# jianzhnie/ScaleRL

Measured on NVIDIA H100. Metric: learner_frames_per_sec, higher is better.
Workload: dtype bf16

## Files before the change

scalerl_b200/csrc/igemm_tma.cuh:

```cuda
#pragma once
#include <cuda.h>
#include "common.cuh"
#include "kernels.h"

namespace srl {

SRL_DEVINL void tma_prefetch_desc(const CUtensorMap* m) {
  asm volatile("prefetch.tensormap [%0];" ::"l"(reinterpret_cast<uint64_t>(m)) : "memory");
}
SRL_DEVINL void tma_load_2d(void* dst, const CUtensorMap* m, uint64_t* bar, int c0, int c1) {
  asm volatile("cp.async.bulk.tensor.2d.shared::cluster.global.mbarrier::complete_tx::bytes [%0], [%1, {%3, %4}], [%2];"
               ::"r"(smem_u32(dst)), "l"(reinterpret_cast<uint64_t>(m)), "r"(smem_u32(bar)), "r"(c0), "r"(c1) : "memory");
}
SRL_DEVINL void tma_load_3d(void* dst, const CUtensorMap* m, uint64_t* bar, int c0, int c1, int c2) {
  asm volatile("cp.async.bulk.tensor.3d.shared::cluster.global.mbarrier::complete_tx::bytes [%0], [%1, {%3, %4, %5}], [%2];"
               ::"r"(smem_u32(dst)), "l"(reinterpret_cast<uint64_t>(m)), "r"(smem_u32(bar)), "r"(c0), "r"(c1), "r"(c2) : "memory");
}
SRL_DEVINL void tma_load_4d(void* dst, const CUtensorMap* m, uint64_t* bar, int c0, int c1, int c2, int c3) {
  asm volatile("cp.async.bulk.tensor.4d.shared::cluster.global.mbarrier::complete_tx::bytes [%0], [%1, {%3, %4, %5, %6}], [%2];"
               ::"r"(smem_u32(dst)), "l"(reinterpret_cast<uint64_t>(m)), "r"(smem_u32(bar)), "r"(c0), "r"(c1), "r"(c2), "r"(c3)
               : "memory");
}
SRL_DEVINL void tma_load_5d(void* dst, const CUtensorMap* m, uint64_t* bar, int c0, int c1, int c2, int c3, int c4) {
  asm volatile("cp.async.bulk.tensor.5d.shared::cluster.global.mbarrier::complete_tx::bytes [%0], [%1, {%3, %4, %5, %6, %7}], [%2];"
               ::"r"(smem_u32(dst)), "l"(reinterpret_cast<uint64_t>(m)), "r"(smem_u32(bar)), "r"(c0), "r"(c1), "r"(c2), "r"(c3), "r"(c4)
               : "memory");
}

constexpr int IGT_THREADS = 288;

template <class P, int SPLIT = 0>
struct TmaCfg {
  static constexpr int KROWS = P::A_MN ? P::KROWS : 64;
  static constexpr int A_BYTES = P::A_MN ? 2 * KROWS * 128 : 128 * 128;
  static constexpr int B_BLOCKS = (P::BN + 63) / 64;
  static constexpr int B_BYTES = P::B_MN ? B_BLOCKS * KROWS * 128 : P::BN * 128;
  static constexpr int HALF_BYTES = A_BYTES + B_BYTES;
  static constexpr int STAGE_BYTES = HALF_BYTES * (1 + SPLIT);
  static constexpr int NB = P::BN / 2;
  static constexpr int STAGES = fit_stages(P::STAGES, 2 * WG_IMG_BYTES + 1024 + 256, STAGE_BYTES);
  static constexpr int SMEM_BYTES = STAGES * STAGE_BYTES + 2 * WG_IMG_BYTES + 1024 + 256;
  static_assert(SMEM_BYTES <= 232448, "shared memory budget (227 KB)");
  static_assert(NB == 32 || NB == 64 || NB == 128, "MMA N per warpgroup");
  static constexpr int MMAS = P::A_MN ? KROWS / 16 : 4;
  static_assert(A_BYTES % 1024 == 0 && B_BYTES % 1024 == 0, "operand tiles must keep 1024 B alignment (SWIZZLE_128B atoms)");
  static_assert(P::A_MN == P::B_MN, "mixed majors are not used");
  static_assert(KROWS % 16 == 0, "contraction rows per stage must be a multiple of MMA K = 16");
};

template <class P, int SPLIT>
SRL_DEVINL void igt_epilogue(const typename P::Params& p, int tm, int ty, int row, int c0, float (&v)[16]) {
  if constexpr (SPLIT) P::template epilogue16<1>(p, tm, ty, row, c0, v); else P::epilogue16(p, tm, ty, row, c0, v);
}
template <class P, int SPLIT>
SRL_DEVINL void igt_epilogue(const typename P::Params& p, int tm, int ty, int row, int c0, float (&v)[16], const uint4 (&pre)[2]) {
  if constexpr (SPLIT) P::template epilogue16<1>(p, tm, ty, row, c0, v, pre); else P::epilogue16(p, tm, ty, row, c0, v, pre);
}

template <class P, int SPLIT = 0>
__global__ void __launch_bounds__(IGT_THREADS) igemm_tma_kernel(const __grid_constant__ typename P::Params p) {
  using C = TmaCfg<P, SPLIT>;
  extern __shared__ uint8_t smem_raw[];
  uint8_t* smem = reinterpret_cast<uint8_t*>((reinterpret_cast<uintptr_t>(smem_raw) + 1023) & ~uintptr_t(1023));
  float* img = reinterpret_cast<float*>(smem + C::STAGES * C::STAGE_BYTES);
  uint64_t* bars = reinterpret_cast<uint64_t*>(smem + C::STAGES * C::STAGE_BYTES + 2 * WG_IMG_BYTES);
  uint64_t* full = bars;
  uint64_t* empty = bars + C::STAGES;

  const int tid = threadIdx.x;
  const int warp = tid >> 5;
  const int tm = blockIdx.x, ty = blockIdx.y;
  const int nkb = P::num_kblocks(p, tm, ty);

  if constexpr (P::ZERO_INIT) {
    if (P::zero_cta(ty)) {
      uint4* z = reinterpret_cast<uint4*>(smem);
      for (int i = tid; i < C::STAGES * C::STAGE_BYTES / 16; i += IGT_THREADS) z[i] = make_uint4(0, 0, 0, 0);
    }
    __syncthreads();
    for (int s = 0; s < C::STAGES; ++s) P::init_smem(p, tm, ty, smem + s * C::STAGE_BYTES, tid);
    fence_proxy_async_smem();
  }
  if (warp == 8 && (tid & 31) == 0) {
    for (int s = 0; s < C::STAGES; ++s) { mbar_init(&full[s], 1); mbar_init(&empty[s], 8); }
    mbar_fence_init();
    P::prefetch(p);
  }
  __syncthreads();
  pdl_wait(P::KID);
  if (tid == 256) pdl_launch();

  if (warp == 8) {
    const uint32_t leader = elect_one_sync();
    for (int kb = 0; kb < nkb; ++kb) {
      const int s = kb % C::STAGES;
      mbar_wait(&empty[s], ((kb / C::STAGES) & 1) ^ 1);
      if (leader) {
        uint8_t* sA = smem + s * C::STAGE_BYTES;
        if constexpr (SPLIT) P::issue_split(p, tm, ty, kb, sA, C::A_BYTES, C::HALF_BYTES, &full[s]);
        else P::issue(p, tm, ty, kb, sA, sA + C::A_BYTES, &full[s]);
      }
      __syncwarp();
    }
  } else {
    const int g = warp >> 2, wt = tid & 127;
    constexpr int NB = C::NB;
    uint4 pre[P::PREFETCH ? NB / 16 : 1][2];
    if constexpr (P::PREFETCH) {
#pragma unroll
      for (int c = 0; c < NB / 16; ++c) P::prefetch16(p, tm, ty, wt, g * NB + c * 16, pre[c]);
    }
    float acc[2][NB / 2];
#pragma unroll
    for (int h = 0; h < 2; ++h)
#pragma unroll
      for (int i = 0; i < NB / 2; ++i) acc[h][i] = 0.f;
    constexpr uint32_t ASTEP = P::A_MN ? 2048 / 16 : 32 / 16, BSTEP = P::B_MN ? 2048 / 16 : 32 / 16;
    constexpr uint32_t A_HI = (P::A_MN ? C::KROWS * 128 : 64 * 128) / 16;
    const uint32_t b_off = P::B_MN ? (g * NB / 64) * C::KROWS * 128 + (g * NB % 64) * 2 : g * NB * 128;
    for (int kb = 0; kb < nkb; ++kb) {
      const int s = kb % C::STAGES;
      mbar_wait(&full[s], (kb / C::STAGES) & 1);
      const uint32_t a0 = smem_u32(smem + s * C::STAGE_BYTES);
      const uint64_t ad0 = P::A_MN ? make_smem_desc(a0, C::KROWS * 128, 1024) : make_smem_desc(a0, 16, 1024);
      const uint64_t bd0 = P::B_MN ? make_smem_desc(a0 + C::A_BYTES + b_off, C::KROWS * 128, 1024) : make_smem_desc(a0 + C::A_BYTES + b_off, 16, 1024);
      wg_fence();
#pragma unroll
      for (int k = 0; k < C::MMAS; ++k) {
        const uint64_t ad = ad0 + (uint64_t)(k * ASTEP), bd = bd0 + (uint64_t)(k * BSTEP);
        wg_mma128<NB, P::A_MN ? 1 : 0, P::B_MN ? 1 : 0>(acc, ad, A_HI, bd, (kb | k) != 0);
        if constexpr (SPLIT) {
          wg_mma128<NB, P::A_MN ? 1 : 0, P::B_MN ? 1 : 0>(acc, ad, A_HI, bd + (uint64_t)(C::HALF_BYTES / 16), 1);
          wg_mma128<NB, P::A_MN ? 1 : 0, P::B_MN ? 1 : 0>(acc, ad + (uint64_t)(C::HALF_BYTES / 16), A_HI, bd, 1);
        }
      }
      wg_commit();
      if constexpr (C::STAGES > 1) {
        wg_wait_prev();
        __syncwarp();
        if (kb > 0 && (tid & 31) == 0) mbar_arrive(&empty[(kb - 1) % C::STAGES]);
      } else {
        wg_wait_all();
        __syncwarp();
        if ((tid & 31) == 0) mbar_arrive(&empty[s]);
      }
    }
    wg_wait_all();
    wg_fence_regs(acc[0]); wg_fence_regs(acc[1]);
    float* my_img = img + g * (WG_IMG_BYTES / 4);
#pragma unroll
    for (int c = 0; c < NB / 16; ++c) {
      float v[16];
      wg_acc_row16<NB>(acc, c, my_img, wt, 2 + g, v);
      if constexpr (P::PREFETCH) igt_epilogue<P, SPLIT>(p, tm, ty, wt, g * NB + c * 16, v, pre[c]);
      else igt_epilogue<P, SPLIT>(p, tm, ty, wt, g * NB + c * 16, v);
    }
  }
}

template <class P, int SPLIT = 0>
cudaError_t igemm_tma_launch(const typename P::Params& p, dim3 grid, cudaStream_t stream) {
  using C = TmaCfg<P, SPLIT>;
  if (grid.x == 0 || grid.y == 0) return cudaSuccess;
  static PerDeviceOnce once;
  { cudaError_t e = ensure_max_dynamic_smem(once, igemm_tma_kernel<P, SPLIT>, C::SMEM_BYTES); if (e != cudaSuccess) return e; }
  return launch_chain(igemm_tma_kernel<P, SPLIT>, grid, dim3(IGT_THREADS), C::SMEM_BYTES, stream, p);
}

}
```

scalerl_b200/csrc/tma_problems.cuh:

```cuda
#pragma once
#include "igemm_tma.cuh"
#include "encoder_problems.cuh"

namespace srl {

#define SRL_TMAP alignas(64) CUtensorMap

struct TFcFwd {
  static constexpr int KID = 31;
  static constexpr bool PREFETCH = false;
  static constexpr int BN = 64, STAGES = 4, SPLITS = 4;
  static constexpr bool A_MN = false, B_MN = false, ZERO_INIT = false;
  static constexpr int KROWS = 64;
  struct Params { SRL_TMAP a3m; SRL_TMAP w; SRL_TMAP a3m_lo; SRL_TMAP w_lo; float* out; int M; };
  SRL_DEVINL static void prefetch(const Params& p) { tma_prefetch_desc(&p.a3m); tma_prefetch_desc(&p.w); }
  SRL_DEVINL static int kb_begin(int split) { return (49 * split) / SPLITS; }
  SRL_DEVINL static void issue_split(const Params& p, int tm, int ty, int kb, uint8_t* st, int a_bytes, int half, uint64_t* bar) {
    const int k = (kb_begin(ty % SPLITS) + kb) * 64;
    mbar_arrive_expect_tx(bar, 2 * (128 * 128 + 64 * 128));
    tma_load_2d(st, &p.a3m, bar, k, tm * 128);
    tma_load_2d(st + a_bytes, &p.w, bar, k, (ty / SPLITS) * 64);
    tma_load_2d(st + half, &p.a3m_lo, bar, k, tm * 128);
    tma_load_2d(st + half + a_bytes, &p.w_lo, bar, k, (ty / SPLITS) * 64);
  }
  template <int SPLIT>
  SRL_DEVINL static void epilogue16(const Params& p, int tm, int ty, int row, int c0, float (&v)[16]) { epilogue16(p, tm, ty, row, c0, v); }
  SRL_DEVINL static int num_kblocks(const Params&, int, int ty) { const int sp = ty % SPLITS; return kb_begin(sp + 1) - kb_begin(sp); }
  SRL_DEVINL static void issue(const Params& p, int tm, int ty, int kb, uint8_t* sA, uint8_t* sB, uint64_t* bar) {
    const int k = (kb_begin(ty % SPLITS) + kb) * 64;
    mbar_arrive_expect_tx(bar, 128 * 128 + 64 * 128);
    tma_load_2d(sA, &p.a3m, bar, k, tm * 128);
    tma_load_2d(sB, &p.w, bar, k, (ty / SPLITS) * 64);
  }
  SRL_DEVINL static void epilogue16(const Params& p, int tm, int ty, int row, int c0, float (&v)[16]) {
    const int m = tm * 128 + row;
    if (m >= p.M) return;
    float4* o = reinterpret_cast<float4*>(p.out + ((size_t)(ty % SPLITS) * p.M + m) * 512 + (ty / SPLITS) * 64 + c0);
#pragma unroll
    for (int j = 0; j < 4; ++j) o[j] = make_float4(v[4 * j], v[4 * j + 1], v[4 * j + 2], v[4 * j + 3]);
  }
};

struct TFcDgrad {
  static constexpr int KID = 32;
  static constexpr bool PREFETCH = true;
  static constexpr int BN = 64, STAGES = 4;
  static constexpr bool A_MN = false, B_MN = false, ZERO_INIT = false;
  static constexpr int KROWS = 64;
  struct Params { SRL_TMAP dhm; SRL_TMAP w; SRL_TMAP dhm_lo; SRL_TMAP w_lo; const bf16* a3; bf16* da3; bf16* da3_lo; int M; };
  SRL_DEVINL static void prefetch(const Params& p) { tma_prefetch_desc(&p.dhm); tma_prefetch_desc(&p.w); }
  SRL_DEVINL static int num_kblocks(const Params&, int, int) { return 8; }
  SRL_DEVINL static void issue_split(const Params& p, int tm, int ty, int kb, uint8_t* st, int a_bytes, int half, uint64_t* bar) {
    mbar_arrive_expect_tx(bar, 2 * (128 * 128 + 64 * 128));
    tma_load_2d(st, &p.dhm, bar, kb * 64, tm * 128);
    tma_load_2d(st + a_bytes, &p.w, bar, kb * 64, ty * 64);
    tma_load_2d(st + half, &p.dhm_lo, bar, kb * 64, tm * 128);
    tma_load_2d(st + half + a_bytes, &p.w_lo, bar, kb * 64, ty * 64);
  }
  SRL_DEVINL static void issue(const Params& p, int tm, int ty, int kb, uint8_t* sA, uint8_t* sB, uint64_t* bar) {
    mbar_arrive_expect_tx(bar, 128 * 128 + 64 * 128);
    tma_load_2d(sA, &p.dhm, bar, kb * 64, tm * 128);
    tma_load_2d(sB, &p.w, bar, kb * 64, ty * 64);
  }
  SRL_DEVINL static void prefetch16(const Params& p, int tm, int ty, int row, int c0, uint4 (&mk)[2]) {
    const int m = tm * 128 + row;
    if (m < p.M) ld_mask16(p.a3 + (size_t)m * 3136 + ty * 64 + c0, mk);
  }
  SRL_DEVINL static void epilogue16(const Params& p, int tm, int ty, int row, int c0, float (&v)[16], const uint4 (&mk)[2]) {
    epilogue16<0>(p, tm, ty, row, c0, v, mk);
  }
  template <int SPLIT>
  SRL_DEVINL static void epilogue16(const Params& p, int tm, int ty, int row, int c0, float (&v)[16], const uint4 (&mk)[2]) {
    const int m = tm * 128 + row;
    if (m >= p.M) return;
    relu_mask16_pre(mk, v);
    const size_t o = ((size_t)m * 81 + (ty / 7) * 9 + ty % 7) * 64 + c0;
    store_bf16x16(p.da3 + o, v);
    if constexpr (SPLIT) {
      float r[16];
#pragma unroll
      for (int j = 0; j < 16; ++j) r[j] = v[j] - __bfloat162float(__float2bfloat16_rn(v[j]));
      store_bf16x16(p.da3_lo + o, r);
    }
  }
};

SRL_DEVINL void fill_ones(uint8_t* dst, int bytes, int tid) {
  uint4* q = reinterpret_cast<uint4*>(dst);
  for (int i = tid; i < bytes / 16; i += IGT_THREADS) q[i] = make_uint4(0x3F803F80u, 0x3F803F80u, 0x3F803F80u, 0x3F803F80u);
}

struct TFcWgrad {
  static constexpr int KID = 33;
  static constexpr bool PREFETCH = false;
  static constexpr int BN = 64, STAGES = 4, KROWS = 64;
  static constexpr bool A_MN = true, B_MN = true, ZERO_INIT = true;
  struct Params { SRL_TMAP dhm; SRL_TMAP a3m; SRL_TMAP dhm_lo; SRL_TMAP a3m_lo; float* dw; float* db; int M; };
  SRL_DEVINL static void prefetch(const Params& p) { tma_prefetch_desc(&p.dhm); tma_prefetch_desc(&p.a3m); }
  SRL_DEVINL static void issue_split(const Params& p, int, int ty, int kb, uint8_t* st, int a_bytes, int half, uint64_t* bar) {
    const int hw = ty >> 2, j0 = (ty & 3) * 128;
    mbar_arrive_expect_tx(bar, (hw < 49 ? 6 : 4) * 64 * 128);
    tma_load_2d(st, &p.dhm, bar, j0, kb * 64);
    tma_load_2d(st + KROWS * 128, &p.dhm, bar, j0 + 64, kb * 64);
    tma_load_2d(st + half, &p.dhm_lo, bar, j0, kb * 64);
    tma_load_2d(st + half + KROWS * 128, &p.dhm_lo, bar, j0 + 64, kb * 64);
    if (hw < 49) {
      tma_load_2d(st + a_bytes, &p.a3m, bar, hw * 64, kb * 64);
      tma_load_2d(st + half + a_bytes, &p.a3m_lo, bar, hw * 64, kb * 64);
    }
  }
  template <int SPLIT>
  SRL_DEVINL static void epilogue16(const Params& p, int tm, int ty, int row, int c0, float (&v)[16]) { epilogue16(p, tm, ty, row, c0, v); }
  SRL_DEVINL static bool zero_cta(int) { return true; }
  SRL_DEVINL static int num_kblocks(const Params& p, int, int) { return (p.M + 63) >> 6; }
  SRL_DEVINL static void init_smem(const Params&, int, int ty, uint8_t* stage, int tid) {
    if ((ty >> 2) == 49) fill_ones(stage + 2 * KROWS * 128, KROWS * 128, tid);
  }
  SRL_DEVINL static void issue(const Params& p, int, int ty, int kb, uint8_t* sA, uint8_t* sB, uint64_t* bar) {
    const int hw = ty >> 2, j0 = (ty & 3) * 128;
    mbar_arrive_expect_tx(bar, (hw < 49 ? 3 : 2) * 64 * 128);
    tma_load_2d(sA, &p.dhm, bar, j0, kb * 64);
    tma_load_2d(sA + KROWS * 128, &p.dhm, bar, j0 + 64, kb * 64);
    if (hw < 49) tma_load_2d(sB, &p.a3m, bar, hw * 64, kb * 64);
  }
  SRL_DEVINL static void epilogue16(const Params& p, int, int ty, int row, int c0, float (&v)[16]) {
    const int j = (ty & 3) * 128 + row, hw = ty >> 2;
    if (hw < 49) {
#pragma unroll
      for (int jj = 0; jj < 16; ++jj) p.dw[(size_t)j * 3136 + (c0 + jj) * 49 + hw] = v[jj];
    } else if (c0 == 0) {
      p.db[j] = v[0];
    }
  }
};

struct TFcWgradN {
  static constexpr int KID = 36;
  static constexpr bool PREFETCH = false;
  static constexpr int BN = 256, STAGES = 4, KROWS = 64, NCT = 13;
  static constexpr bool A_MN = true, B_MN = true, ZERO_INIT = true;
  struct Params { SRL_TMAP dhm; SRL_TMAP a3tm; float* dw; float* db; int M; };
  SRL_DEVINL static void prefetch(const Params& p) { tma_prefetch_desc(&p.dhm); tma_prefetch_desc(&p.a3tm); }
  SRL_DEVINL static bool zero_cta(int ty) { return (ty >> 2) == NCT; }
  SRL_DEVINL static int num_kblocks(const Params& p, int, int) { return (p.M + 63) >> 6; }
  SRL_DEVINL static void init_smem(const Params&, int, int ty, uint8_t* stage, int tid) {
    if ((ty >> 2) == NCT) fill_ones(stage + 2 * KROWS * 128, KROWS * 128, tid);
  }
  SRL_DEVINL static void issue(const Params& p, int, int ty, int kb, uint8_t* sA, uint8_t* sB, uint64_t* bar) {
    const int ct = ty >> 2, j0 = (ty & 3) * 128;
    const int nb = ct < NCT ? (ct == NCT - 1 ? 1 : 4) : 0;
    mbar_arrive_expect_tx(bar, (2 + nb) * 64 * 128);
    tma_load_2d(sA, &p.dhm, bar, j0, kb * 64);
    tma_load_2d(sA + KROWS * 128, &p.dhm, bar, j0 + 64, kb * 64);
    for (int q = 0; q < nb; ++q) tma_load_2d(sB + q * KROWS * 128, &p.a3tm, bar, ct * 256 + q * 64, kb * 64);
  }
  SRL_DEVINL static void epilogue16(const Params& p, int, int ty, int row, int c0, float (&v)[16]) {
    const int j = (ty & 3) * 128 + row, ct = ty >> 2, col = ct * 256 + c0;
    if (ct < NCT) {
      if (col < 3136) {
        float4* d = reinterpret_cast<float4*>(p.dw + (size_t)j * 3136 + col);
#pragma unroll
        for (int q = 0; q < 4; ++q) d[q] = make_float4(v[4 * q], v[4 * q + 1], v[4 * q + 2], v[4 * q + 3]);
      }
    } else if (c0 == 0) {
      p.db[j] = v[0];
    }
  }
};

}
```

Baseline: 2.469 million.

## Halve FC wgrad N-tile and stage accumulators through smem for coalesced stores

The FC weight-gradient GEMM drops its N tile from 256 to 128 columns, roughly doubling the number of column tiles and CTAs. A new tile epilogue path writes each warpgroup's accumulators into a padded shared-memory tile that reuses the stage ring. Threads then emit row-contiguous float4 stores instead of per-thread 16-column row writes. This aims at better SM fill and more coalesced global writes, at the cost of reloading the A operand for more CTAs and an extra smem round trip with barriers.

Measured after the change: 2.488 million (median of 6 runs). About the same (+0.8%).

```diff
diff --git a/scalerl_b200/csrc/igemm_tma.cuh b/scalerl_b200/csrc/igemm_tma.cuh
--- a/scalerl_b200/csrc/igemm_tma.cuh
+++ b/scalerl_b200/csrc/igemm_tma.cuh
@@ -55,6 +55,24 @@
 template <class P, int SPLIT>
 SRL_DEVINL void igt_epilogue(const typename P::Params& p, int tm, int ty, int row, int c0, float (&v)[16], const uint4 (&pre)[2]) {
   if constexpr (SPLIT) P::template epilogue16<1>(p, tm, ty, row, c0, v, pre); else P::epilogue16(p, tm, ty, row, c0, v, pre);
+}
+
+template <class P, class = void> struct IgtTileEpilogue { static constexpr bool value = false; };
+template <class P> struct IgtTileEpilogue<P, decltype((void)&P::epilogue_tile)> { static constexpr bool value = true; };
+template <int NB> constexpr int igt_tile_stride() { return NB + 8; }
+
+template <int N>
+SRL_DEVINL void wg_acc_to_tile(const float (&d)[2][N / 2], float* tile, int stride, int wt) {
+  const int w = wt >> 5, l = wt & 31;
+#pragma unroll
+  for (int h = 0; h < 2; ++h)
+#pragma unroll
+    for (int b = 0; b < N / 8; ++b)
+#pragma unroll
+      for (int rr = 0; rr < 2; ++rr) {
+        const int row = 64 * h + 16 * w + (l >> 2) + 8 * rr, i = 4 * b + 2 * rr;
+        *reinterpret_cast<float2*>(tile + row * stride + 8 * b + 2 * (l & 3)) = make_float2(d[h][i], d[h][i + 1]);
+      }
 }
 
 template <class P, int SPLIT = 0>
@@ -147,13 +165,23 @@
     }
     wg_wait_all();
     wg_fence_regs(acc[0]); wg_fence_regs(acc[1]);
-    float* my_img = img + g * (WG_IMG_BYTES / 4);
+    if constexpr (IgtTileEpilogue<P>::value) {
+      constexpr int STRIDE = igt_tile_stride<NB>();
+      static_assert(2 * 128 * STRIDE * 4 <= C::STAGES * C::STAGE_BYTES + 2 * WG_IMG_BYTES, "staged tile fits the ring + row hand-off buffers");
+      named_bar(1, 256);
+      float* tile = reinterpret_cast<float*>(smem) + g * 128 * STRIDE;
+      wg_acc_to_tile<NB>(acc, tile, STRIDE, wt);
+      named_bar(2 + g, 128);
+      P::epilogue_tile(p, tm, ty, g, wt, tile, STRIDE);
+    } else {
+      float* my_img = img + g * (WG_IMG_BYTES / 4);
 #pragma unroll
-    for (int c = 0; c < NB / 16; ++c) {
-      float v[16];
-      wg_acc_row16<NB>(acc, c, my_img, wt, 2 + g, v);
-      if constexpr (P::PREFETCH) igt_epilogue<P, SPLIT>(p, tm, ty, wt, g * NB + c * 16, v, pre[c]);
-      else igt_epilogue<P, SPLIT>(p, tm, ty, wt, g * NB + c * 16, v);
+      for (int c = 0; c < NB / 16; ++c) {
+        float v[16];
+        wg_acc_row16<NB>(acc, c, my_img, wt, 2 + g, v);
+        if constexpr (P::PREFETCH) igt_epilogue<P, SPLIT>(p, tm, ty, wt, g * NB + c * 16, v, pre[c]);
+        else igt_epilogue<P, SPLIT>(p, tm, ty, wt, g * NB + c * 16, v);
+      }
     }
   }
 }
diff --git a/scalerl_b200/csrc/tma_problems.cuh b/scalerl_b200/csrc/tma_problems.cuh
--- a/scalerl_b200/csrc/tma_problems.cuh
+++ b/scalerl_b200/csrc/tma_problems.cuh
@@ -137,7 +137,7 @@
 struct TFcWgradN {
   static constexpr int KID = 36;
   static constexpr bool PREFETCH = false;
-  static constexpr int BN = 256, STAGES = 4, KROWS = 64, NCT = 13;
+  static constexpr int BN = 128, STAGES = 4, KROWS = 64, NCT = 25;
   static constexpr bool A_MN = true, B_MN = true, ZERO_INIT = true;
   struct Params { SRL_TMAP dhm; SRL_TMAP a3tm; float* dw; float* db; int M; };
   SRL_DEVINL static void prefetch(const Params& p) { tma_prefetch_desc(&p.dhm); tma_prefetch_desc(&p.a3tm); }
@@ -148,23 +148,24 @@
   }
   SRL_DEVINL static void issue(const Params& p, int, int ty, int kb, uint8_t* sA, uint8_t* sB, uint64_t* bar) {
     const int ct = ty >> 2, j0 = (ty & 3) * 128;
-    const int nb = ct < NCT ? (ct == NCT - 1 ? 1 : 4) : 0;
+    const int nb = ct < NCT ? (ct == NCT - 1 ? 1 : 2) : 0;
     mbar_arrive_expect_tx(bar, (2 + nb) * 64 * 128);
     tma_load_2d(sA, &p.dhm, bar, j0, kb * 64);
     tma_load_2d(sA + KROWS * 128, &p.dhm, bar, j0 + 64, kb * 64);
-    for (int q = 0; q < nb; ++q) tma_load_2d(sB + q * KROWS * 128, &p.a3tm, bar, ct * 256 + q * 64, kb * 64);
+    for (int q = 0; q < nb; ++q) tma_load_2d(sB + q * KROWS * 128, &p.a3tm, bar, ct * 128 + q * 64, kb * 64);
   }
-  SRL_DEVINL static void epilogue16(const Params& p, int, int ty, int row, int c0, float (&v)[16]) {
-    const int j = (ty & 3) * 128 + row, ct = ty >> 2, col = ct * 256 + c0;
-    if (ct < NCT) {
-      if (col < 3136) {
-        float4* d = reinterpret_cast<float4*>(p.dw + (size_t)j * 3136 + col);
-#pragma unroll
-        for (int q = 0; q < 4; ++q) d[q] = make_float4(v[4 * q], v[4 * q + 1], v[4 * q + 2], v[4 * q + 3]);
-      }
-    } else if (c0 == 0) {
-      p.db[j] = v[0];
+  SRL_DEVINL static void epilogue_tile(const Params& p, int, int ty, int g, int wt, const float* tile, int stride) {
+    const int ct = ty >> 2, j0 = (ty & 3) * 128;
+    if (ct == NCT) {
+      if (g == 0) p.db[j0 + wt] = tile[wt * stride];
+      return;
     }
+    const int col = ct * 128 + g * 64;
+    if (col >= 3136) return;
+    const int q = wt & 15, r0 = wt >> 4;
+#pragma unroll 4
+    for (int r = r0; r < 128; r += 8)
+      *reinterpret_cast<float4*>(p.dw + (size_t)(j0 + r) * 3136 + col + 4 * q) = *reinterpret_cast<const float4*>(tile + r * stride + 4 * q);
   }
 };
 
```
